# CrawlScript/tf_geometric

Measured on NVIDIA H100. Metric: edges/sec GCN+GAT fwd on 2.4M-node/123M-edge synthetic; %HBM roofline, higher is better.
Workload: dtype f32

## Files before the change

### include/tfgk.h

```cpp
#ifndef TFGK_H_
#define TFGK_H_

#include <stddef.h>
#include <stdint.h>

#ifdef __cplusplus
extern "C" {
#endif

#define TFGK_ABI_VERSION 7

enum tfgk_status {
    TFGK_OK = 0,
    TFGK_ERR_INVALID_ARGUMENT = 1,
    TFGK_ERR_CUDA = 2,
    TFGK_ERR_WORKSPACE = 3,
    TFGK_ERR_UNSUPPORTED = 4,
    TFGK_ERR_INDEX_OUT_OF_RANGE = 5
};

enum tfgk_reduce { TFGK_REDUCE_SUM = 0, TFGK_REDUCE_MEAN = 1, TFGK_REDUCE_MAX = 2 };
enum tfgk_act { TFGK_ACT_NONE = 0, TFGK_ACT_RELU = 1 };
enum tfgk_deg_power { TFGK_POW_INV_SQRT = 0, TFGK_POW_INV = 1 };
enum tfgk_heads_mode { TFGK_HEADS_SPLIT = 0, TFGK_HEADS_BROADCAST = 1, TFGK_HEADS_REDUCE = 2 };
// ... 57 lines not shown


int tfgk_spmm_f32(const int64_t *rowptr, const int32_t *col, const float *w,
                  const float *h, int64_t ldh, int32_t n_dst, int32_t D, int reduce,
                  float alpha, const float *addend, int64_t ld_addend, float beta,
                  const float *bias, int act,
                  float *out, int64_t ldo, const tfgk_plan *plan, void *stream);
int tfgk_spmm_bf16(const int64_t *rowptr, const int32_t *col, const float *w,
                   const uint16_t *h, int64_t ldh, int32_t n_dst, int32_t D, int reduce,
                   float alpha, const float *addend, int64_t ld_addend, float beta,
                   const float *bias, int act,
                   float *out, int64_t ldo, const tfgk_plan *plan, void *stream);
int tfgk_spmm_bf16_dual(const int64_t *rowptr, const int32_t *col, const float *w,
                        const uint16_t *h, int64_t ldh, int32_t n_dst, int32_t D, int reduce,
                        float alpha, const float *addend, int64_t ld_addend, float beta,
                        const float *bias, int act,
                        float *out, int64_t ldo, uint16_t *out_bf16, int64_t ldob,
                        const tfgk_plan *plan, void *stream);


int tfgk_segment_softmax_f32(const int64_t *rowptr, const float *score, int32_t n_seg, int32_t H,
                             float *out, void *stream);

int tfgk_gat_fused_f32(const int64_t *rowptr, const int32_t *col,
                       const float *Q, int64_t ldq, const float *K, int64_t ldk, const float *V, int64_t ldv,
                       int32_t N, int32_t H, int32_t dqk, int32_t dv, float scale, int split_value_heads,
                       const float *bias, int act, float *att, int write_att, float *out, int64_t ldo,
                       const tfgk_plan *plan, void *stream);
int tfgk_gat_fused_bf16(const int64_t *rowptr, const int32_t *col,
                        const float *Q, int64_t ldq, const uint16_t *K, int64_t ldk, const uint16_t *V, int64_t ldv,
                        int32_t N, int32_t H, int32_t dqk, int32_t dv, float scale, int split_value_heads,
                        const float *bias, int act, float *att, int write_att, float *out, int64_t ldo,
                        const tfgk_plan *plan, void *stream);


int tfgk_gemm_workspace_bytes(int32_t M, int32_t N, int32_t K, size_t *out_bytes);
int tfgk_gemm_f32(const float *A, int64_t lda, int transA, const float *B, int64_t ldb, int transB,
                  const float *bias, int act, float beta, int32_t M, int32_t N, int32_t K,
                  float *C, int64_t ldc, void *workspace, size_t workspace_bytes, void *stream);

typedef struct tfgk_proj_block {
    const float *B; int64_t ldb;
    int32_t ncols;
    int32_t transB;
    const float *bias;
    int act;
    float *C; int64_t ldc;
} tfgk_proj_block;
int tfgk_gemm_proj_f32(const float *const *A_parts, int32_t n_parts, int64_t part_rows, int64_t lda,
                       int32_t M, int32_t K, const tfgk_proj_block *blocks, int32_t n_blocks,
                       int32_t first_part, int32_t max_ctas, void *stream);
typedef struct tfgk_proj_block_out {
    const float *B; int64_t ldb;
    int32_t ncols;
    int32_t transB;
    const float *bias;
    int act;
    void *C; int64_t ldc;
    int32_t c_dtype;
} tfgk_proj_block_out;
int tfgk_gemm_proj_mixed(const float *const *A_parts, int32_t n_parts, int64_t part_rows, int64_t lda,
                         int32_t M, int32_t K, const tfgk_proj_block_out *blocks, int32_t n_blocks,
                         int32_t first_part, int32_t max_ctas, void *stream);
int tfgk_round_bf16(const float *src, int64_t lds, int32_t rows, int32_t cols, uint16_t *dst, int64_t ldd, void *stream);

#define TFGK_PEER_HANDLE_BYTES 64
// ... 125 lines not shown
```

### tf_geometric_b200/_ffi.py

```python
import ctypes
import os
import threading

_LIB_PATH = os.path.join(os.path.dirname(os.path.abspath(__file__)), "lib", "libtfgk.so")
_lock = threading.Lock()
_lib = None

ABI_VERSION = 7

OK = 0
ERR_INVALID_ARGUMENT, ERR_CUDA, ERR_WORKSPACE, ERR_UNSUPPORTED, ERR_INDEX_OUT_OF_RANGE = 1, 2, 3, 4, 5
REDUCE_SUM, REDUCE_MEAN, REDUCE_MAX = 0, 1, 2
ACT_NONE, ACT_RELU = 0, 1
POW_INV_SQRT, POW_INV = 0, 1
HEADS_SPLIT, HEADS_BROADCAST, HEADS_REDUCE = 0, 1, 2
FLAG_ALL, FLAG_UPPER, FLAG_MAPPED = 0, 1, 2
BERNOULLI_NONE, BERNOULLI_DROPOUT, BERNOULLI_KEEP = 0, 1, 2
SAMPLE_NO_PADDING, SAMPLE_PADDING, SAMPLE_HEAD = 0, 1, 2
NEG_UPPER, NEG_START = 0, 1
PAD_ROW_MAJOR, PAD_STEP_MAJOR = 0, 1
DTYPE_F32, DTYPE_BF16 = 0, 1

_i32, _i64, _f32, _int = ctypes.c_int32, ctypes.c_int64, ctypes.c_float, ctypes.c_int
_ptr, _size = ctypes.c_void_p, ctypes.c_size_t
# ... 1 lines not shown

SIGNATURES = {
    "tfgk_version": [],
    "tfgk_device_info": [ctypes.POINTER(_int)] * 3,
    "tfgk_self_loops_i32": [_ptr, _i64, _i32, _ptr, _ptr],
    "tfgk_self_loop_weights_f32": [_ptr, _i64, _i32, _f32, _ptr, _ptr],
    "tfgk_segment_count_i32": [_ptr, _i64, _i32, _ptr, _ptr],
    "tfgk_csr_workspace_bytes": [_i64, _i32, ctypes.POINTER(_size)],
    "tfgk_csr_build": [_ptr, _ptr, _i64, _i32, _i32, _ptr, _ptr, _ptr, _ptr, _size, _ptr],
    "tfgk_edge_unique_workspace_bytes": [_i64, _i32, ctypes.POINTER(_size)],
    "tfgk_edge_unique": [_ptr, _ptr, _i64, _i32, _ptr, _ptr, ctypes.POINTER(_i32), _ptr, _size, _ptr],
    "tfgk_directed_workspace_bytes": [_i64, ctypes.POINTER(_size)],
    "tfgk_directed_edges": [_ptr, _i64, _i64, _ptr, _i64, _ptr, ctypes.POINTER(_i32), _ptr, _size, _ptr],
    "tfgk_plan_capacity": [_i64, _i32, _i32, _i32, _i32, ctypes.POINTER(_i64), ctypes.POINTER(_i64)],
    "tfgk_plan_workspace_bytes": [_i32, ctypes.POINTER(_size)],
    "tfgk_plan_build": [_ptr, _i32, _i32, _i32, _i32, _ptr, _ptr, _ptr, _ptr, _ptr, _ptr, _ptr, _ptr, _i64, _i64,
                        ctypes.POINTER(_i32), _ptr, _size, _ptr],
    "tfgk_permute_f32": [_ptr, _ptr, _i64, _i32, _ptr, _ptr],
    "tfgk_unpermute_f32": [_ptr, _ptr, _i64, _i32, _ptr, _ptr],
    "tfgk_csr_rowsum_f32": [_ptr, _ptr, _i32, _ptr, _ptr],
    "tfgk_deg_inv_f32": [_ptr, _i32, _int, _ptr, _ptr],
    "tfgk_scale_edges_f32": [_ptr, _ptr, _ptr, _i64, _ptr, _ptr, _ptr, _ptr],
    "tfgk_spmm_f32": [_ptr, _ptr, _ptr, _ptr, _i64, _i32, _i32, _int, _f32, _ptr, _i64, _f32, _ptr, _int, _ptr, _i64,
                      _ptr, _ptr],
    "tfgk_spmm_bf16": [_ptr, _ptr, _ptr, _ptr, _i64, _i32, _i32, _int, _f32, _ptr, _i64, _f32, _ptr, _int, _ptr, _i64,
                       _ptr, _ptr],
    "tfgk_spmm_bf16_dual": [_ptr, _ptr, _ptr, _ptr, _i64, _i32, _i32, _int, _f32, _ptr, _i64, _f32, _ptr, _int, _ptr,
                            _i64, _ptr, _i64, _ptr, _ptr],
    "tfgk_segment_softmax_f32": [_ptr, _ptr, _i32, _i32, _ptr, _ptr],
    "tfgk_gat_fused_f32": [_ptr, _ptr, _ptr, _i64, _ptr, _i64, _ptr, _i64, _i32, _i32, _i32, _i32, _f32, _int, _ptr,
                           _int, _ptr, _int, _ptr, _i64, _ptr, _ptr],
    "tfgk_gat_fused_bf16": [_ptr, _ptr, _ptr, _i64, _ptr, _i64, _ptr, _i64, _i32, _i32, _i32, _i32, _f32, _int, _ptr,
                            _int, _ptr, _int, _ptr, _i64, _ptr, _ptr],
    "tfgk_gemm_workspace_bytes": [_i32, _i32, _i32, ctypes.POINTER(_size)],
    "tfgk_gemm_f32": [_ptr, _i64, _int, _ptr, _i64, _int, _ptr, _int, _f32, _i32, _i32, _i32, _ptr, _i64, _ptr, _size,
                      _ptr],
    "tfgk_gemm_proj_f32": [_ptr, _i32, _i64, _i64, _i32, _i32, _ptr, _i32, _i32, _i32, _ptr],
    "tfgk_gemm_proj_mixed": [_ptr, _i32, _i64, _i64, _i32, _i32, _ptr, _i32, _i32, _i32, _ptr],
    "tfgk_round_bf16": [_ptr, _i64, _i32, _i32, _ptr, _i64, _ptr],
    "tfgk_peer_alloc": [_size, ctypes.POINTER(_ptr)],
    "tfgk_peer_free": [_ptr],
    "tfgk_peer_export": [_ptr, _ptr],
    "tfgk_peer_open": [_ptr, ctypes.POINTER(_ptr)],
    "tfgk_peer_close": [_ptr],
    "tfgk_peer_barrier": [_ptr, _i32, _i32, _u32, _i32, _ptr],
    "tfgk_peer_pull": [_ptr, _ptr, _i64, _i32, _ptr],
    "tfgk_colsum_workspace_bytes": [_i64, _i32, ctypes.POINTER(_size)],
    "tfgk_colsum_f32": [_ptr, _i64, _i64, _i32, _ptr, _ptr, _size, _ptr],
    "tfgk_l2_normalize_f32": [_ptr, _i64, _i32, _i32, _ptr, _i64, _ptr],
    "tfgk_dropout_f32": [_ptr, _i64, _f32, _u64, _u32, _ptr, _ptr],
    "tfgk_spmm_heads_f32": [_ptr, _ptr, _ptr, _ptr, _ptr, _i64, _i32, _i32, _i32, _int, _f32, _u64, _u32, _f32, _ptr,
                            _int, _ptr, _i64, _ptr],
    "tfgk_gat_softmax_bwd_f32": [_ptr, _ptr, _ptr, _ptr, _i64, _ptr, _i64, _i32, _i32, _i32, _int, _f32, _u64, _u32,
                                 _ptr, _ptr],
    "tfgk_gat_fused_stats_f32": [_ptr, _ptr, _ptr, _i64, _ptr, _i64, _ptr, _i64, _i32, _i32, _i32, _i32, _f32, _ptr, _int,
                                 _ptr, _i64, _ptr, _ptr, _ptr],
    "tfgk_gat_bwd_prepare_f32": [_ptr, _i64, _ptr, _i64, _ptr, _int, _ptr, _i32, _i32, _i32, _ptr, _i64, _ptr],
    "tfgk_gat_bwd_dst_f32": [_ptr, _ptr, _ptr, _i64, _ptr, _i64, _ptr, _i64, _ptr, _i64, _i32, _i32, _i32, _f32, _ptr, _i64,
                             _ptr],
    "tfgk_gat_bwd_src_f32": [_ptr, _ptr, _ptr, _i64, _ptr, _i64, _ptr, _i64, _ptr, _i64, _i32, _i32, _i32, _f32, _ptr, _i64,
                             _ptr, _i64, _ptr],
    "tfgk_edge_flags_i32": [_ptr, _ptr, _i64, _int, _ptr, _ptr, _int, _f32, _u64, _u32, _ptr, _ptr],
    "tfgk_select_workspace_bytes": [_i64, ctypes.POINTER(_size)],
    "tfgk_select_flagged_i32": [_ptr, _i64, _ptr, ctypes.POINTER(_i64), _ptr, _size, _ptr],
    "tfgk_sort_keys_f32": [_ptr, _i64, _int, _ptr, _ptr],
    "tfgk_argsort_workspace_bytes": [_i64, ctypes.POINTER(_size)],
# ... 120 lines not shown
```

### tf_geometric_b200/csrc/gat.cu

```cuda
#include "common.cuh"
#include <stdlib.h>
#include <string.h>

namespace tfgk {

constexpr int kGatThreads = 256;
constexpr int kGatWarps = kGatThreads / 32;
constexpr int kMaxHeadsFast = 32;

__device__ __forceinline__ float4 ldg4(const float *p) { return __ldg(reinterpret_cast<const float4 *>(p)); }
__device__ __forceinline__ float4 ldg_row4(const float *p) { return ldg4(p); }
__device__ __forceinline__ float4 ldg_row4(const uint16_t *p) {
    const uint2 t = __ldg(reinterpret_cast<const uint2 *>(p));
    return make_float4(bf16_to_f32(t.x & 0xFFFFu), bf16_to_f32(t.x >> 16), bf16_to_f32(t.y & 0xFFFFu), bf16_to_f32(t.y >> 16));
}

struct GatParams {
    const int64_t *rowptr;
    const int32_t *col;
    const float *Q; int64_t ldq;
    const float *K; int64_t ldk;
    const float *V; int64_t ldv;
    const uint16_t *Kb, *Vb;
    int32_t N, H, dqk, dv;
    float scale;
    int split;
    const float *bias;
    int act;
    float *att;
    int write_att;
    float *out; int64_t ldo;
    int32_t n_tasks;
    const int32_t *task_row, *task_nrows;
    const int64_t *task_e0, *task_e1;
    const int32_t *task_slot;
    int32_t n_hubs;
    const int32_t *hub_row, *hub_slot0, *hub_nslots;
    float *scratch;
    float *stats;
};

template <int NCK, int NCV, int U>
__global__ void __launch_bounds__(kGatThreads) gat_fast_kernel(const GatParams p) {
    __shared__ float s_max[kGatWarps][kMaxHeadsFast];
    __shared__ float s_den[kGatWarps][kMaxHeadsFast];
    const int lane = threadIdx.x & 31, warp = threadIdx.x >> 5;
    const int64_t r = (int64_t)blockIdx.x * kGatWarps + warp;
    if (r >= p.N) return;
    const int H = p.H;
    const int A = H * p.dqk, VW = H * p.dv;
    const int lanes_per_head = p.dqk >> 2;
    const int64_t start = p.rowptr[r];
    const int deg = (int)(p.rowptr[r + 1] - start);
    float *att = p.att + start * H;

    int kcol[NCK];
    bool kok[NCK];
    float4 q[NCK];
    float mx[NCK];
#pragma unroll
    for (int k = 0; k < NCK; ++k) {
        kcol[k] = (lane + 32 * k) * 4;
        kok[k] = kcol[k] < A;
        q[k] = kok[k] ? ldg4(p.Q + r * p.ldq + kcol[k]) : make_float4(0.f, 0.f, 0.f, 0.f);
        mx[k] = -FLT_MAX;
    }
    for (int t = 0; t < deg; t += 32) {
        const int e = t + lane;
        const int my_c = e < deg ? ld_stream_i32(p.col + start + e) : 0;
        const int nb = min(32, deg - t);
        for (int j = 0; j < nb; j += U) {
            float4 kk[U][NCK];
// ... 595 lines not shown
        return TFGK_ERR_UNSUPPORTED;
    const size_t stage_pitch = ((size_t)4 * 2 * A * sizeof(T) + 127) & ~(size_t)127;
    const size_t smem = (size_t)kGatAsyncWarps * S * stage_pitch + (size_t)kGatAsyncWarps * S * 8;
    TFGK_CUDA(ensure_dynamic_smem(gat_tma4_kernel<S, T>, smem));
    const int64_t n_tasks = p.task_row ? p.n_tasks : ceil_div64(p.N, kGatAsyncRows);
    const unsigned blocks = (unsigned)ceil_div64(n_tasks, kGatAsyncWarps);
    gat_tma4_kernel<S, T><<<blocks, kGatAsyncWarps * 32, smem, st>>>(p);
    TFGK_LAUNCH_CHECK();
    if (p.task_row && p.n_hubs > 0) {
        gat_hub_fixup_kernel<<<(unsigned)ceil_div64(p.n_hubs, 8), 256, 0, st>>>(p);
        TFGK_LAUNCH_CHECK();
    }
    return TFGK_OK;
}

static int dispatch_gat_async(const GatParams &p, cudaStream_t st) {
    const char *g4 = getenv("TFGK_GAT_IMPL");
    if (!(g4 && g4[0] == 'a')) {
        const char *colon = g4 ? strchr(g4, ':') : nullptr;
        const int stages = colon ? atoi(colon + 1) : 2;
        const int rc = stages == 2 ? launch_gat_tma4<2>(p, st) : stages == 4 ? launch_gat_tma4<4>(p, st)
                                                                           : launch_gat_tma4<3>(p, st);
        if (rc != TFGK_ERR_UNSUPPORTED) return rc;
    }
    const char *cfg = getenv("TFGK_GAT_ASYNC_CFG");
    if (cfg && cfg[0] == '4' && cfg[2] == '2') return launch_gat_async<4, 2>(p, st);
    if (cfg && cfg[0] == '4' && cfg[2] == '3') return launch_gat_async<4, 3>(p, st);
    if (cfg && cfg[0] == '2' && cfg[2] == '4') return launch_gat_async<2, 4>(p, st);
    if (cfg && cfg[0] == '2' && cfg[2] == '2') return launch_gat_async<2, 2>(p, st);
    if (cfg && cfg[0] == '1' && cfg[2] == '4') return launch_gat_async<1, 4>(p, st);
    return launch_gat_async<2, 3>(p, st);
}

__device__ __forceinline__ float warp_sum(float v) {
#pragma unroll
    for (int off = 16; off > 0; off >>= 1) v += __shfl_xor_sync(0xffffffffu, v, off);
    return v;
}
__device__ __forceinline__ float warp_max(float v) {
#pragma unroll
    for (int off = 16; off > 0; off >>= 1) v = fmaxf(v, __shfl_xor_sync(0xffffffffu, v, off));
    return v;
}

__device__ __forceinline__ float ld_elem(const float *p) { return *p; }
__device__ __forceinline__ float ld_elem(const uint16_t *p) { return bf16_to_f32(*p); }

template <typename T>
__global__ void __launch_bounds__(kGatThreads) gat_generic_kernel(const GatParams p) {
    const T *Kt = sizeof(T) == 4 ? (const T *)p.K : (const T *)p.Kb;
    const T *Vt = sizeof(T) == 4 ? (const T *)p.V : (const T *)p.Vb;
    extern __shared__ float smem[];
    const int lane = threadIdx.x & 31, warp = threadIdx.x >> 5;
    const int64_t r = (int64_t)blockIdx.x * kGatWarps + warp;
    if (r >= p.N) return;
    const int H = p.H;
    float *s_max = smem + (size_t)warp * 2 * H;
    float *s_den = s_max + H;
    const int64_t start = p.rowptr[r];
    const int deg = (int)(p.rowptr[r + 1] - start);
    float *att = p.att + start * H;
    const int32_t *col = p.col + start;

    for (int h = lane; h < H; h += 32) s_max[h] = -FLT_MAX;
    __syncwarp();
    for (int e = 0; e < deg; ++e) {
// ... 240 lines not shown
    if (plan != nullptr && plan->n_tasks > 0) {
        if (plan->n_hubs > 0)
            TFGK_CHECK_ARG(plan->scratch != nullptr && plan->scratch_bytes >= (size_t)plan->n_slots * (VW + 64) * sizeof(float),
                           "gat: plan scratch too small (need %zu bytes)", (size_t)plan->n_slots * (VW + 64) * sizeof(float));
        p.n_tasks = plan->n_tasks; p.task_row = plan->task_row; p.task_nrows = plan->task_nrows;
        p.task_e0 = plan->task_e0; p.task_e1 = plan->task_e1; p.task_slot = plan->task_slot;
        p.n_hubs = plan->n_hubs; p.hub_row = plan->hub_row; p.hub_slot0 = plan->hub_slot0;
        p.hub_nslots = plan->hub_nslots; p.scratch = plan->scratch;
    }
    cudaStream_t st = as_stream(stream);
    const bool fast = split_value_heads && is_pow2(H) && H <= kMaxHeadsFast && dqk == dv && dqk % 4 == 0 &&
                      is_pow2(dqk / 4) && dqk <= 128 && A <= 512 && ldq % 4 == 0 && ldk % 4 == 0 && ldv % 4 == 0 &&
                      ldo % 4 == 0 && aligned16(Q) && aligned8(K) && aligned8(V) && aligned16(out) &&
                      (!bias || aligned16(bias));
    if (fast && A <= 128) {
        const int rc = launch_gat_tma4<3, uint16_t>(p, st);
        if (rc != TFGK_ERR_UNSUPPORTED) return rc;
    }
    if (fast) {
        switch ((A + 127) / 128) {
            case 1: return launch_gat_online<1, uint16_t>(p, st);
            case 2: return launch_gat_online<2, uint16_t>(p, st);
            case 3: return launch_gat_online<3, uint16_t>(p, st);
            default: return launch_gat_online<4, uint16_t>(p, st);
        }
    }
    if (att == nullptr) return set_error(TFGK_ERR_WORKSPACE, "gat: this shape needs the [E,H] attention scratch buffer");
    const size_t smem = (size_t)kGatWarps * 2 * H * sizeof(float);
    TFGK_CHECK_ARG(smem <= 48 * 1024, "gat: too many heads for the generic path (H=%d)", H);
    gat_generic_kernel<uint16_t><<<(unsigned)ceil_div64(N, kGatWarps), kGatThreads, smem, st>>>(p);
    TFGK_LAUNCH_CHECK();
    return TFGK_OK;
}
```

### tf_geometric_b200/nn/conv/gat.py

```python
import torch

from ... import ops, _structure, _rng, autograd
from ...sparse import as_sparse_features, project_features


def project(x, blocks):
    pieces = []
    for w, b, act, out in blocks:
        for c0 in range(0, w.shape[1], 128):
            c1 = min(c0 + 128, w.shape[1])
            pieces.append((w[:, c0:c1], None if b is None else b[c0:c1], act, out[:, c0:c1]))
    for i in range(0, len(pieces), 4):
        ops.gemm_proj(x, pieces[i:i + 4])


def gat(x, edge_index,
        query_kernel, query_bias, query_activation,
        key_kernel, key_bias, key_activation,
        kernel, bias=None, activation=None, num_heads=1,
        split_value_heads=True, edge_drop_rate=0.0, training=False, cache=None, return_attention=False, seed=None,
        message_dtype=None):
    bf16 = ops.message_dtype(message_dtype) is not None
    if bf16:
        if as_sparse_features(x) is not None:
            raise NotImplementedError("message_dtype=bfloat16 takes a dense x")
        if training and edge_drop_rate > 0.0:
            raise NotImplementedError("message_dtype=bfloat16 is for inference: attention dropout is not applied in bf16")
        if return_attention:
            raise NotImplementedError("message_dtype=bfloat16 does not return attention coefficients")
    edge_index = ops.as_device(edge_index, torch.int32)
    dev = edge_index.device
    x_sparse = as_sparse_features(x)
# ... 8 lines not shown
                raise NotImplementedError("return_attention is an inference-path extension")
            return _gat_training(x_sparse, csr, edge_index_used, query_kernel, query_bias, query_activation, key_kernel,
                                 key_bias, key_activation, kernel, bias, activation, num_heads, split_value_heads, drop_rate,
                                 _rng.resolve(seed) if drop_rate > 0.0 else 0)
        q_act, q_left = ops.activation_code(query_activation)
        k_act, k_left = ops.activation_code(key_activation)
        f32 = lambda t: None if t is None else ops.as_device(t, torch.float32, device=dev)
        Q = project_features(x_sparse, query_kernel, bias=f32(query_bias), act=q_act)
        K = project_features(x_sparse, key_kernel, bias=f32(key_bias), act=k_act)
        V = project_features(x_sparse, kernel)
        Q = q_left(Q) if q_left is not None else Q
        K = k_left(K) if k_left is not None else K
        act_code, leftover = ops.activation_code(activation)
        res = ops.gat_fused(csr, Q, K, V, num_heads, split_value_heads=split_value_heads, bias=f32(bias), act=act_code,
                            return_attention=return_attention)
        h, att = res if return_attention else (res, None)
        h = leftover(h) if leftover is not None else h
        return (h, ops.permute(att, csr.perm, inverse=True)) if return_attention else h
    if drop_rate > 0.0 or autograd.needs_grad(x, query_kernel, query_bias, key_kernel, key_bias, kernel, bias):
        if bf16:
            raise NotImplementedError("message_dtype=bfloat16 is for inference: no operand may require grad")
        if return_attention:
            raise NotImplementedError("return_attention is an inference-path extension")
        return _gat_training(x, csr, edge_index_used, query_kernel, query_bias, query_activation, key_kernel, key_bias,
                             key_activation, kernel, bias, activation, num_heads, split_value_heads, drop_rate,
                             _rng.resolve(seed) if drop_rate > 0.0 else 0)

    q_act, q_left = ops.activation_code(query_activation)
    k_act, k_left = ops.activation_code(key_activation)
    wq = ops.as_device(query_kernel, torch.float32, device=dev)
    wk = ops.as_device(key_kernel, torch.float32, device=dev)
    wv = ops.as_device(kernel, torch.float32, device=dev)
    a_units = wk.shape[1]
    Q = torch.empty((num_nodes, wq.shape[1]), dtype=torch.float32, device=dev)
    kv = torch.empty((num_nodes, a_units + wv.shape[1]), dtype=torch.bfloat16 if bf16 else torch.float32, device=dev)
    K, V = kv[:, :a_units], kv[:, a_units:]
    K_f32 = torch.empty((num_nodes, a_units), dtype=torch.float32, device=dev) if bf16 and k_left is not None else K
    project(x, [(wq, ops.as_device(query_bias, torch.float32, device=dev), q_act, Q),
                (wk, ops.as_device(key_bias, torch.float32, device=dev), k_act, K_f32),
                (wv, None, ops.ACT_NONE, V)])
    if q_left is not None:
        Q = q_left(Q)
    if k_left is not None:
        if K_f32 is K:
            K.copy_(k_left(K))
        else:
            ops.round_bf16(k_left(K_f32), out=K)

    act_code, leftover = ops.activation_code(activation)
    bias = None if bias is None else ops.as_device(bias, torch.float32, device=dev)
    res = ops.gat_fused(csr, Q, K, V, num_heads, split_value_heads=split_value_heads, bias=bias, act=act_code,
                        return_attention=return_attention)
    h, att = res if return_attention else (res, None)
    if leftover is not None:
        h = leftover(h)
    if return_attention:
        return h, ops.permute(att, csr.perm, inverse=True)
    return h


def _gat_training(x, csr, edge_index_used, query_kernel, query_bias, query_activation, key_kernel, key_bias,
                  key_activation, kernel, bias, activation, num_heads, split_value_heads, drop_rate, seed):
    sparse_x = as_sparse_features(x)
    dev = csr.col.device

    def dense(w, b, act):
        code, left = ops.activation_code(act)
        w = ops.as_device(w, torch.float32, device=dev)
        b = None if b is None else ops.as_device(b, torch.float32, device=dev)
        y = autograd.Dense.apply(x, w, b, code) if sparse_x is None else autograd.SparseMatmul.apply(w, b, sparse_x, code)
        return left(y) if left is not None else y

    Q = dense(query_kernel, query_bias, query_activation)
    K = dense(key_kernel, key_bias, key_activation)
    V = dense(kernel, None, None)
    act_code, leftover = ops.activation_code(activation)
    bias = None if bias is None else ops.as_device(bias, torch.float32, device=dev)
    h = autograd.GatAttention.apply(Q, K, V, bias, csr, edge_index_used, int(num_heads), bool(split_value_heads),
                                    act_code, drop_rate, seed)
    return leftover(h) if leftover is not None else h
```

### tf_geometric_b200/ops.py

```python
import ctypes

import numpy as np
import torch

from . import _ffi
from ._ffi import (REDUCE_SUM, REDUCE_MEAN, REDUCE_MAX, ACT_NONE, ACT_RELU, POW_INV_SQRT, POW_INV,
                   HEADS_SPLIT, HEADS_BROADCAST, HEADS_REDUCE, FLAG_ALL, FLAG_UPPER, FLAG_MAPPED,
                   BERNOULLI_NONE, BERNOULLI_DROPOUT, BERNOULLI_KEEP, SAMPLE_NO_PADDING, SAMPLE_PADDING, SAMPLE_HEAD,
                   NEG_UPPER, NEG_START, PAD_ROW_MAJOR, PAD_STEP_MAJOR)

_REDUCE_CODES = {"sum": REDUCE_SUM, "mean": REDUCE_MEAN, "max": REDUCE_MAX}


def _require_cuda():
    if not torch.cuda.is_available():
        raise RuntimeError("tf_geometric_b200 needs a CUDA device (H100 / sm_90a); there is no CPU fallback")


def default_device():
    _require_cuda()
    return torch.device("cuda", torch.cuda.current_device())


def as_device(x, dtype=None, device=None):
# ... 297 lines not shown
        raise ValueError("attention units ({}) and value units ({}) must be divisible by num_heads ({})".format(A, VW, H))
    dqk, dv = A // H, VW // H
    out_w = VW if split_value_heads else dv
    if out is None:
        out = torch.empty((N, out_w), dtype=torch.float32, device=Q.device)
    att = att_buffer
    if att is not None and att.numel() < csr.nnz * H:
        att = None
    if att is None and return_attention:
        att = torch.empty((csr.nnz, H), dtype=torch.float32, device=Q.device)
    if bias is not None:
        _check(bias, torch.float32, "bias")
    scale = float(np.sqrt(np.float32(dqk))) if scale is None else float(scale)

    plan = getattr(csr, "plan", None)
    plan_struct = plan.struct(VW + 64, Q.device) if plan is not None else None

    def launch(att_buf):
        _ffi.call("tfgk_gat_fused_bf16" if bf16 else "tfgk_gat_fused_f32", _p(csr.rowptr), _p(csr.col), _p(Q),
                  _row_major_2d(Q, "Q"), _p(K),
                  _row_major_2d(K, "K"), _p(V), _row_major_2d(V, "V"), N, H, dqk, dv, scale,
                  1 if split_value_heads else 0, _p(bias), act, _p(att_buf), 1 if return_attention else 0, _p(out),
                  _row_major_2d(out, "out"), ctypes.byref(plan_struct) if plan_struct is not None else None, _stream(Q))

    try:
        launch(att)
    except _ffi.TfgkError as err:
        if err.code != _ffi.ERR_WORKSPACE or att is not None:
            raise
        att = torch.empty((csr.nnz, H), dtype=torch.float32, device=Q.device)
        launch(att)
    if return_attention:
        return out, att[:csr.nnz]
    return out


def gat_fused_stats(csr, Q, K, V, num_heads, bias=None, act=ACT_NONE, scale=None):
    N, H = csr.n_rows, int(num_heads)
    A = Q.shape[1]
    if A % H or V.shape[1] != A or K.shape[1] != A:
        return None
    dqk = A // H
    scale = float(np.sqrt(np.float32(dqk))) if scale is None else float(scale)
    out = torch.empty((N, A), dtype=torch.float32, device=Q.device)
    stats = torch.empty((N, 2 * H), dtype=torch.float32, device=Q.device)
    plan = getattr(csr, "plan", None)
    plan_struct = plan.struct(A + 64, Q.device) if plan is not None else None
    try:
        _ffi.call("tfgk_gat_fused_stats_f32", _p(csr.rowptr), _p(csr.col), _p(Q), _row_major_2d(Q, "Q"), _p(K),
                  _row_major_2d(K, "K"), _p(V), _row_major_2d(V, "V"), N, H, dqk, dqk, scale, _p(bias), act, _p(out),
                  _row_major_2d(out, "out"), _p(stats), ctypes.byref(plan_struct) if plan_struct is not None else None, _stream(Q))
    except _ffi.TfgkError as err:
        if err.code != _ffi.ERR_UNSUPPORTED:
            raise
        return None
    return out, stats


def gat_backward_recompute(csr, csr_t, Q, K, V, G, Y, bias, act, stats, num_heads, scale):
    N, H = csr.n_rows, int(num_heads)
    A = Q.shape[1]
    dqk = A // H
    GS = torch.empty((N, A + 32), dtype=torch.float32, device=Q.device)
    dQ, dK, dV = torch.empty_like(Q), torch.empty_like(K), torch.empty_like(V)
    try:
        _ffi.call("tfgk_gat_bwd_prepare_f32", _p(G), _row_major_2d(G, "G"), _p(Y), _row_major_2d(Y, "Y"), _p(bias), act,
# ... 512 lines not shown
```

Measured before the change: 3.580 billion.

## Add sparsity-packed key table for GAT with ReLU keys to cut gather bytes

When keys pass through ReLU, a new pack kernel stores each node's V row followed by a nonzero bitmask and a compacted list of the nonzero K values, plus a per-node size byte. A new TMA-ring GAT kernel fetches only that variable-length slot per neighbor and rebuilds K from the mask with popcounts. The aim is to shrink the bytes gathered per edge, which dominate this bandwidth-bound kernel. It adds a pack pass, a per-edge size lookup, and decode work in the inner loop, and it only helps when ReLU leaves many keys at zero.

```diff
diff --git a/include/tfgk.h b/include/tfgk.h
--- a/include/tfgk.h
+++ b/include/tfgk.h
@@ -113,6 +113,12 @@
                         int32_t N, int32_t H, int32_t dqk, int32_t dv, float scale, int split_value_heads,
                         const float *bias, int act, float *att, int write_att, float *out, int64_t ldo,
                         const tfgk_plan *plan, void *stream);
+int tfgk_gat_pack_keys_f32(const float *K, int64_t ldk, int32_t N, int32_t A, float *table, int64_t ldt, uint8_t *ksize,
+                           void *stream);
+int tfgk_gat_fused_packed_f32(const int64_t *rowptr, const int32_t *col, const float *Q, int64_t ldq,
+                              const float *table, int64_t ldt, const uint8_t *ksize, int32_t N, int32_t H, int32_t dqk,
+                              float scale, const float *bias, int act, float *out, int64_t ldo,
+                              const tfgk_plan *plan, void *stream);
 
 
 int tfgk_gemm_workspace_bytes(int32_t M, int32_t N, int32_t K, size_t *out_bytes);
diff --git a/tf_geometric_b200/_ffi.py b/tf_geometric_b200/_ffi.py
--- a/tf_geometric_b200/_ffi.py
+++ b/tf_geometric_b200/_ffi.py
@@ -57,6 +57,9 @@
                            _int, _ptr, _int, _ptr, _i64, _ptr, _ptr],
     "tfgk_gat_fused_bf16": [_ptr, _ptr, _ptr, _i64, _ptr, _i64, _ptr, _i64, _i32, _i32, _i32, _i32, _f32, _int, _ptr,
                             _int, _ptr, _int, _ptr, _i64, _ptr, _ptr],
+    "tfgk_gat_pack_keys_f32": [_ptr, _i64, _i32, _i32, _ptr, _i64, _ptr, _ptr],
+    "tfgk_gat_fused_packed_f32": [_ptr, _ptr, _ptr, _i64, _ptr, _i64, _ptr, _i32, _i32, _i32, _f32, _ptr, _int, _ptr, _i64,
+                                  _ptr, _ptr],
     "tfgk_gemm_workspace_bytes": [_i32, _i32, _i32, ctypes.POINTER(_size)],
     "tfgk_gemm_f32": [_ptr, _i64, _int, _ptr, _i64, _int, _ptr, _int, _f32, _i32, _i32, _i32, _ptr, _i64, _ptr, _size,
                       _ptr],
diff --git a/tf_geometric_b200/csrc/gat.cu b/tf_geometric_b200/csrc/gat.cu
--- a/tf_geometric_b200/csrc/gat.cu
+++ b/tf_geometric_b200/csrc/gat.cu
@@ -38,6 +38,7 @@
     const int32_t *hub_row, *hub_slot0, *hub_nslots;
     float *scratch;
     float *stats;
+    const uint8_t *ksize = nullptr;
 };
 
 template <int NCK, int NCV, int U>
@@ -699,6 +700,234 @@
     return launch_gat_async<2, 3>(p, st);
 }
 
+constexpr int kPackWarps = 8;
+
+__global__ void __launch_bounds__(kPackWarps * 32) gat_pack_keys_kernel(const float *__restrict__ K, int64_t ldk, int32_t N,
+                                                                       int32_t A, float *__restrict__ table, int64_t ldt,
+                                                                       uint8_t *__restrict__ ksize) {
+    const int lane = threadIdx.x & 31;
+    const int64_t n = (int64_t)blockIdx.x * kPackWarps + (threadIdx.x >> 5);
+    if (n >= N) return;
+    const int ccol = lane * 4;
+    const float4 k = ccol < A ? __ldg(reinterpret_cast<const float4 *>(K + n * ldk + ccol)) : make_float4(0.f, 0.f, 0.f, 0.f);
+    const uint32_t nib = (__float_as_uint(k.x) != 0u ? 1u : 0u) | (__float_as_uint(k.y) != 0u ? 2u : 0u) |
+                         (__float_as_uint(k.z) != 0u ? 4u : 0u) | (__float_as_uint(k.w) != 0u ? 8u : 0u);
+    uint32_t word = nib << ((lane & 7) * 4);
+    word |= __shfl_xor_sync(0xffffffffu, word, 1);
+    word |= __shfl_xor_sync(0xffffffffu, word, 2);
+    word |= __shfl_xor_sync(0xffffffffu, word, 4);
+    const int cnt = __popc(nib);
+    int incl = cnt;
+#pragma unroll
+    for (int off = 1; off < 32; off <<= 1) {
+        const int t = __shfl_up_sync(0xffffffffu, incl, off);
+        if (lane >= off) incl += t;
+    }
+    const int total = __shfl_sync(0xffffffffu, incl, 31);
+    const uint32_t m0 = __shfl_sync(0xffffffffu, word, 0), m1 = __shfl_sync(0xffffffffu, word, 8);
+    const uint32_t m2 = __shfl_sync(0xffffffffu, word, 16), m3 = __shfl_sync(0xffffffffu, word, 24);
+    float *slot = table + n * ldt;
+    if (lane == 0) *reinterpret_cast<uint4 *>(slot + A) = make_uint4(m0, m1, m2, m3);
+    float *packed = slot + A + 4;
+    int o = incl - cnt;
+    if (nib & 1u) packed[o++] = k.x;
+    if (nib & 2u) packed[o++] = k.y;
+    if (nib & 4u) packed[o++] = k.z;
+    if (nib & 8u) packed[o] = k.w;
+    const int padded = (total + 3) & ~3;
+    if (lane < padded - total) packed[total + lane] = 0.0f;
+    if (lane == 0) ksize[n] = (uint8_t)((A + 4 + padded) / 4);
+}
+
+template <int S>
+__global__ void __launch_bounds__(kGatAsyncWarps * 32) gat_tma4_packed_kernel(const GatParams p) {
+    constexpr int U = 4, RPC = 32 / U;
+    static_assert(S - 1 <= RPC / 2, "the prologue must not reach the round that fetches chunk 1's copy sizes");
+    extern __shared__ __align__(128) uint8_t gat_pk_ring[];
+    const int lane = threadIdx.x & 31, warp = threadIdx.x >> 5;
+    const int A = p.H * p.dqk;
+    const uint32_t row_bytes = (uint32_t)A * 4u;
+    const uint32_t slot_bytes = (2u * row_bytes + 16u + 127u) & ~127u;
+    const uint32_t stage_bytes = (U * slot_bytes + 127u) & ~127u;
+    uint8_t *my_ring = gat_pk_ring + (size_t)warp * S * stage_bytes;
+    const uint32_t ring_addr = (uint32_t)__cvta_generic_to_shared(my_ring);
+    uint64_t *bars = reinterpret_cast<uint64_t *>(gat_pk_ring + (size_t)kGatAsyncWarps * S * stage_bytes) + warp * S;
+    const uint32_t bar0 = (uint32_t)__cvta_generic_to_shared(bars);
+    if (lane == 0) {
+#pragma unroll
+        for (int i = 0; i < S; ++i) asm volatile("mbarrier.init.shared::cta.b64 [%0], 1;" ::"r"(bar0 + 8 * i));
+        asm volatile("fence.mbarrier_init.release.cluster;" ::: "memory");
+    }
+    __syncwarp();
+    const int64_t task = (int64_t)blockIdx.x * kGatAsyncWarps + warp;
+    int64_t r0, r1, e_begin, e_stop;
+    int slot = -1;
+    if (p.task_row != nullptr) {
+        if (task >= p.n_tasks) return;
+        r0 = p.task_row[task];
+        r1 = r0 + p.task_nrows[task];
+        e_begin = p.task_e0[task];
+        e_stop = p.task_e1[task];
+        slot = p.task_slot[task];
+    } else {
+        r0 = task * kGatAsyncRows;
+        if (r0 >= p.N) return;
+        r1 = min((int64_t)p.N, r0 + kGatAsyncRows);
+        e_begin = p.rowptr[r0];
+        e_stop = p.rowptr[r1];
+    }
+    const int64_t rp_hi = p.rowptr[min(r0 + lane + 1, r1)];
+    const int n_edges = (int)(e_stop - e_begin);
+    const int n_rounds = (n_edges + U - 1) / U;
+    const int lanes_per_head = p.dqk >> 2;
+    const int ccol = lane * 4;
+    const bool cok = ccol < A;
+    const int sh = (lane & 7) * 4, wsel = lane >> 3;
+    const uint32_t below_lo = (1u << sh) - 1u;
+    const uint32_t bm0 = wsel > 0 ? ~0u : wsel == 0 ? below_lo : 0u, bm1 = wsel > 1 ? ~0u : wsel == 1 ? below_lo : 0u;
+    const uint32_t bm2 = wsel > 2 ? ~0u : wsel == 2 ? below_lo : 0u, bm3 = wsel == 3 ? below_lo : 0u;
+
+    int64_t r = r0;
+    int row_end = slot >= 0 ? 0x7fffffff : (int)(__shfl_sync(0xffffffffu, rp_hi, 0) - e_begin);
+    float4 q = cok ? ldg4(p.Q + r * p.ldq + ccol) : make_float4(0.f, 0.f, 0.f, 0.f);
+    float4 q_next = (cok && r + 1 < r1) ? ldg4(p.Q + (r + 1) * p.ldq + ccol) : make_float4(0.f, 0.f, 0.f, 0.f);
+    float mx = -FLT_MAX, den = 0.0f, a0 = 0.f, a1 = 0.f, a2 = 0.f, a3 = 0.f;
+    float4 bias = make_float4(0.f, 0.f, 0.f, 0.f);
+    if (p.bias && cok) bias = ldg4(p.bias + ccol);
+
+    auto finalize_row = [&]() {
+        if (cok) {
+            const float inv = 1.0f / (den + 1e-8f);
+            float4 o;
+            o.x = apply_act(a0 * inv + bias.x, p.act);
+            o.y = apply_act(a1 * inv + bias.y, p.act);
+            o.z = apply_act(a2 * inv + bias.z, p.act);
+            o.w = apply_act(a3 * inv + bias.w, p.act);
+            *reinterpret_cast<float4 *>(p.out + r * p.ldo + ccol) = o;
+        }
+        mx = -FLT_MAX; den = 0.0f; a0 = a1 = a2 = a3 = 0.0f;
+        ++r;
+        q = q_next;
+        if (r < r1) {
+            row_end = (int)(__shfl_sync(0xffffffffu, rp_hi, (int)(r - r0)) - e_begin);
+            if (cok && r + 1 < r1) q_next = ldg4(p.Q + (r + 1) * p.ldq + ccol);
+        }
+    };
+    auto load_chunk = [&](int c) {
+        const int e = c * 32 + lane;
+        return e < n_edges ? ld_stream_i32(p.col + e_begin + e) : 0;
+    };
+    auto load_sizes = [&](int ci) { return (int)__ldg(p.ksize + ci); };
+    auto issue = [&](int g, int ci, int si) {
+        if (g < n_rounds) {
+            const int base = (g % RPC) * U;
+            const int valid = min(U, n_edges - g * U);
+            const int src = base + (lane < U ? lane : 0);
+            const int c = __shfl_sync(0xffffffffu, ci, src);
+            const uint32_t bytes = 16u * (uint32_t)__shfl_sync(0xffffffffu, si, src);
+            uint32_t tx = lane < valid ? bytes : 0u;
+            tx += __shfl_xor_sync(0xffffffffu, tx, 1);
+            tx += __shfl_xor_sync(0xffffffffu, tx, 2);
+            const uint32_t bar = bar0 + 8 * (uint32_t)(g % S);
+            if (lane == 0)
+                asm volatile("mbarrier.arrive.expect_tx.shared::cta.b64 _, [%0], %1;" ::"r"(bar), "r"(tx) : "memory");
+            if (lane < valid)
+                asm volatile("cp.async.bulk.shared::cluster.global.mbarrier::complete_tx::bytes [%0], [%1], %2, [%3];"
+                             ::"r"(ring_addr + (uint32_t)(g % S) * stage_bytes + (uint32_t)lane * slot_bytes),
+                             "l"(p.K + (int64_t)c * p.ldk), "r"(bytes), "r"(bar) : "memory");
+        }
+    };
+
+    int ca = load_chunk(0), cb = load_chunk(1);
+    int sa = load_sizes(ca), sb = 0;
+#pragma unroll
+    for (int g = 0; g < S - 1; ++g) issue(g, ca, sa);
+
+    for (int g = 0; g < n_rounds; ++g) {
+        __syncwarp();
+        {
+            const int gn = g + S - 1;
+            const int k = gn / RPC;
+            if (gn % RPC == RPC / 2) {
+                if (k & 1) sa = load_sizes(ca); else sb = load_sizes(cb);
+            }
+            issue(gn, (k & 1) ? cb : ca, (k & 1) ? sb : sa);
+        }
+        gat_mbar_wait(bar0 + 8 * (uint32_t)(g % S), (uint32_t)(g / S) & 1u);
+        const uint8_t *sbuf = my_ring + (size_t)(g % S) * stage_bytes;
+        float4 kr[U];
+#pragma unroll
+        for (int u = 0; u < U; ++u) {
+            kr[u] = make_float4(0.f, 0.f, 0.f, 0.f);
+            if (g * U + u < n_edges && cok) {
+                const uint8_t *sl = sbuf + (size_t)u * slot_bytes + row_bytes;
+                const uint4 m = *reinterpret_cast<const uint4 *>(sl);
+                const uint32_t bits = *reinterpret_cast<const uint32_t *>(sl + 4 * wsel) >> sh;
+                int o = __popc(m.x & bm0) + __popc(m.y & bm1) + __popc(m.z & bm2) + __popc(m.w & bm3);
+                const float *pk = reinterpret_cast<const float *>(sl + 16);
+                if (bits & 1u) kr[u].x = pk[o++];
+                if (bits & 2u) kr[u].y = pk[o++];
+                if (bits & 4u) kr[u].z = pk[o++];
+                if (bits & 8u) kr[u].w = pk[o];
+            }
+        }
+#pragma unroll
+        for (int u = 0; u < U; ++u) {
+            const int e = g * U + u;
+            if (e < n_edges) {
+                while (e == row_end) finalize_row();
+                const float4 kk = kr[u];
+                float4 vv = make_float4(0.f, 0.f, 0.f, 0.f);
+                if (cok) vv = *reinterpret_cast<const float4 *>(sbuf + (size_t)u * slot_bytes + ccol * 4);
+                float d = __fmul_rn(q.x, kk.x);
+                d = fmaf(q.y, kk.y, d);
+                d = fmaf(q.z, kk.z, d);
+                d = fmaf(q.w, kk.w, d);
+                for (int off = 1; off < lanes_per_head; off <<= 1) d += __shfl_xor_sync(0xffffffffu, d, off);
+                const float s = __fdiv_rn(d, p.scale);
+                const bool up = s > mx;
+                const float t = expf(up ? mx - s : s - mx);
+                const float corr = up ? t : 1.0f, pe = up ? 1.0f : t;
+                mx = up ? s : mx;
+                den = fmaf(den, corr, pe);
+                a0 = fmaf(a0, corr, pe * vv.x);
+                a1 = fmaf(a1, corr, pe * vv.y);
+                a2 = fmaf(a2, corr, pe * vv.z);
+                a3 = fmaf(a3, corr, pe * vv.w);
+            }
+        }
+        if ((g + S) % RPC == 0) {
+            const int dead = (g + S) / RPC - 1;
+            if (dead & 1) cb = load_chunk(dead + 2); else ca = load_chunk(dead + 2);
+        }
+    }
+    if (slot >= 0) {
+        float *dst = p.scratch + (int64_t)slot * (A + 64);
+        if (cok) *reinterpret_cast<float4 *>(dst + ccol) = make_float4(a0, a1, a2, a3);
+        dst[A + lane] = mx;
+        dst[A + 32 + lane] = den;
+        return;
+    }
+    while (r < r1) finalize_row();
+}
+
+template <int S>
+static int launch_gat_packed(const GatParams &p, cudaStream_t st) {
+    const size_t slot_bytes = ((size_t)8 * p.H * p.dqk + 16 + 127) & ~(size_t)127;
+    const size_t stage_pitch = (4 * slot_bytes + 127) & ~(size_t)127;
+    const size_t smem = (size_t)kGatAsyncWarps * S * stage_pitch + (size_t)kGatAsyncWarps * S * 8;
+    TFGK_CUDA(ensure_dynamic_smem(gat_tma4_packed_kernel<S>, smem));
+    const int64_t n_tasks = p.task_row ? p.n_tasks : ceil_div64(p.N, kGatAsyncRows);
+    const unsigned blocks = (unsigned)ceil_div64(n_tasks, kGatAsyncWarps);
+    gat_tma4_packed_kernel<S><<<blocks, kGatAsyncWarps * 32, smem, st>>>(p);
+    TFGK_LAUNCH_CHECK();
+    if (p.task_row && p.n_hubs > 0) {
+        gat_hub_fixup_kernel<<<(unsigned)ceil_div64(p.n_hubs, 8), 256, 0, st>>>(p);
+        TFGK_LAUNCH_CHECK();
+    }
+    return TFGK_OK;
+}
+
 __device__ __forceinline__ float warp_sum(float v) {
 #pragma unroll
     for (int off = 16; off > 0; off >>= 1) v += __shfl_xor_sync(0xffffffffu, v, off);
@@ -1005,3 +1234,59 @@
     TFGK_LAUNCH_CHECK();
     return TFGK_OK;
 }
+
+extern "C" int tfgk_gat_pack_keys_f32(const float *K, int64_t ldk, int32_t N, int32_t A, float *table, int64_t ldt,
+                                      uint8_t *ksize, void *stream) {
+    TFGK_CHECK_ARG(N >= 0 && A >= 4 && A <= 128 && A % 4 == 0, "gat_pack_keys: bad size (N=%d A=%d; A must be 4..128, a multiple of 4)",
+                   N, A);
+    TFGK_CHECK_ARG(ldk >= A && ldk % 4 == 0 && ldt >= 2 * A + 4 && ldt % 16 == 0,
+                   "gat_pack_keys: leading dimensions (ldk=%lld, ldt=%lld; ldt a multiple of 16, at least 2A + 4)",
+                   (long long)ldk, (long long)ldt);
+    if (N == 0) return TFGK_OK;
+    TFGK_CHECK_ARG(K && table && ksize, "gat_pack_keys: null pointer");
+    TFGK_CHECK_ARG(aligned16(K) && aligned16(table), "gat_pack_keys: K and table must be 16-byte aligned");
+    gat_pack_keys_kernel<<<(unsigned)ceil_div64(N, kPackWarps), kPackWarps * 32, 0, as_stream(stream)>>>(K, ldk, N, A, table,
+                                                                                                         ldt, ksize);
+    TFGK_LAUNCH_CHECK();
+    return TFGK_OK;
+}
+
+extern "C" int tfgk_gat_fused_packed_f32(const int64_t *rowptr, const int32_t *col, const float *Q, int64_t ldq,
+                                         const float *table, int64_t ldt, const uint8_t *ksize, int32_t N, int32_t H,
+                                         int32_t dqk, float scale, const float *bias, int act, float *out, int64_t ldo,
+                                         const tfgk_plan *plan, void *stream) {
+    TFGK_CHECK_ARG(N >= 0 && H >= 1 && dqk >= 1, "gat_packed: bad size (N=%d H=%d dqk=%d)", N, H, dqk);
+    TFGK_CHECK_ARG(act == TFGK_ACT_NONE || act == TFGK_ACT_RELU, "gat_packed: unknown activation %d", act);
+    TFGK_CHECK_ARG(scale > 0.0f, "gat_packed: scale must be positive");
+    const int A = H * dqk;
+    if (!(is_pow2(H) && H <= kMaxHeadsFast && dqk % 4 == 0 && is_pow2(dqk / 4) && A <= 128))
+        return set_error(TFGK_ERR_UNSUPPORTED, "gat_packed: H must be a power of two <= 32, dqk / 4 a power of two, H * dqk <= 128");
+    TFGK_CHECK_ARG(ldq >= A && ldo >= A && ldt >= 2 * A + 4, "gat_packed: leading dimension too small");
+    if (N == 0) return TFGK_OK;
+    TFGK_CHECK_ARG(rowptr && col && Q && table && ksize && out, "gat_packed: null pointer");
+    if (ldq % 4 || ldo % 4 || ldt % 16 || !aligned16(Q) || !aligned16(out) || !aligned16(table) || (bias && !aligned16(bias)))
+        return set_error(TFGK_ERR_UNSUPPORTED, "gat_packed: Q, out, bias and table need 16-byte aligned rows, slots of a multiple of 64 bytes");
+
+    GatParams p;
+    p.rowptr = rowptr; p.col = col;
+    p.Q = Q; p.ldq = ldq; p.K = table; p.ldk = ldt; p.V = table; p.ldv = ldt; p.Kb = nullptr; p.Vb = nullptr;
+    p.N = N; p.H = H; p.dqk = dqk; p.dv = dqk; p.scale = scale; p.split = 1;
+    p.bias = bias; p.act = act; p.att = nullptr; p.write_att = 0; p.out = out; p.ldo = ldo;
+    p.n_tasks = 0; p.task_row = nullptr; p.task_nrows = nullptr; p.task_e0 = nullptr; p.task_e1 = nullptr;
+    p.task_slot = nullptr; p.n_hubs = 0; p.hub_row = nullptr; p.hub_slot0 = nullptr; p.hub_nslots = nullptr; p.scratch = nullptr;
+    p.stats = nullptr;
+    p.ksize = ksize;
+    if (plan != nullptr && plan->n_tasks > 0) {
+        if (plan->n_hubs > 0)
+            TFGK_CHECK_ARG(plan->scratch != nullptr && plan->scratch_bytes >= (size_t)plan->n_slots * (A + 64) * sizeof(float),
+                           "gat_packed: plan scratch too small (need %zu bytes)", (size_t)plan->n_slots * (A + 64) * sizeof(float));
+        p.n_tasks = plan->n_tasks; p.task_row = plan->task_row; p.task_nrows = plan->task_nrows;
+        p.task_e0 = plan->task_e0; p.task_e1 = plan->task_e1; p.task_slot = plan->task_slot;
+        p.n_hubs = plan->n_hubs; p.hub_row = plan->hub_row; p.hub_slot0 = plan->hub_slot0;
+        p.hub_nslots = plan->hub_nslots; p.scratch = plan->scratch;
+    }
+    cudaStream_t st = as_stream(stream);
+    const char *env = getenv("TFGK_GAT_PACKED_STAGES");
+    const int stages = env ? atoi(env) : 2;
+    return stages == 3 ? launch_gat_packed<3>(p, st) : stages == 4 ? launch_gat_packed<4>(p, st) : launch_gat_packed<2>(p, st);
+}
diff --git a/tf_geometric_b200/nn/conv/gat.py b/tf_geometric_b200/nn/conv/gat.py
--- a/tf_geometric_b200/nn/conv/gat.py
+++ b/tf_geometric_b200/nn/conv/gat.py
@@ -1,3 +1,5 @@
+import os
+
 import torch
 
 from ... import ops, _structure, _rng, autograd
@@ -72,6 +74,24 @@
     wk = ops.as_device(key_kernel, torch.float32, device=dev)
     wv = ops.as_device(kernel, torch.float32, device=dev)
     a_units = wk.shape[1]
+    act_code, leftover = ops.activation_code(activation)
+    bias = None if bias is None else ops.as_device(bias, torch.float32, device=dev)
+    if not bf16 and not return_attention and k_act == ops.ACT_RELU and k_left is None and x.is_cuda and \
+            _packed_keys_shape(wq, wk, wv, bias, num_heads, split_value_heads) and \
+            os.environ.get("TFGK_GAT_KEYS", "packed") != "dense":
+        Q = torch.empty((num_nodes, a_units), dtype=torch.float32, device=dev)
+        K = torch.empty((num_nodes, a_units), dtype=torch.float32, device=dev)
+        table, sizes = ops.packed_key_table(num_nodes, a_units, dev)
+        project(x, [(wq, ops.as_device(query_bias, torch.float32, device=dev), q_act, Q),
+                    (wk, ops.as_device(key_bias, torch.float32, device=dev), k_act, K),
+                    (wv, None, ops.ACT_NONE, table[:, :a_units])])
+        if q_left is not None:
+            Q = q_left(Q)
+        ops.gat_pack_keys(K, table, sizes)
+        del K
+        h = ops.gat_fused_packed(csr, Q, table, sizes, num_heads, bias=bias, act=act_code)
+        return leftover(h) if leftover is not None else h
+
     Q = torch.empty((num_nodes, wq.shape[1]), dtype=torch.float32, device=dev)
     kv = torch.empty((num_nodes, a_units + wv.shape[1]), dtype=torch.bfloat16 if bf16 else torch.float32, device=dev)
     K, V = kv[:, :a_units], kv[:, a_units:]
@@ -87,8 +107,6 @@
         else:
             ops.round_bf16(k_left(K_f32), out=K)
 
-    act_code, leftover = ops.activation_code(activation)
-    bias = None if bias is None else ops.as_device(bias, torch.float32, device=dev)
     res = ops.gat_fused(csr, Q, K, V, num_heads, split_value_heads=split_value_heads, bias=bias, act=act_code,
                         return_attention=return_attention)
     h, att = res if return_attention else (res, None)
@@ -97,6 +115,14 @@
     if return_attention:
         return h, ops.permute(att, csr.perm, inverse=True)
     return h
+
+
+def _packed_keys_shape(wq, wk, wv, bias, num_heads, split_value_heads):
+    H, A = int(num_heads), wk.shape[1]
+    if not split_value_heads or wq.shape[1] != A or wv.shape[1] != A or A > 128 or H < 1 or H > 32 or H & (H - 1) or A % H:
+        return False
+    d4 = (A // H) // 4
+    return (A // H) % 4 == 0 and d4 >= 1 and d4 & (d4 - 1) == 0 and (bias is None or bias.data_ptr() % 16 == 0)
 
 
 def _gat_training(x, csr, edge_index_used, query_kernel, query_bias, query_activation, key_kernel, key_bias,
diff --git a/tf_geometric_b200/ops.py b/tf_geometric_b200/ops.py
--- a/tf_geometric_b200/ops.py
+++ b/tf_geometric_b200/ops.py
@@ -353,6 +353,48 @@
         launch(att)
     if return_attention:
         return out, att[:csr.nnz]
+    return out
+
+
+def gat_packed_width(units):
+    return -(-(2 * int(units) + 4) // 32) * 32
+
+
+def packed_key_table(num_nodes, units, device):
+    table = torch.empty((int(num_nodes), gat_packed_width(units)), dtype=torch.float32, device=device)
+    sizes = torch.empty((int(num_nodes),), dtype=torch.uint8, device=device)
+    return table, sizes
+
+
+def gat_pack_keys(K, table, sizes):
+    if not (K.is_cuda and K.dtype == torch.float32 and K.dim() == 2):
+        raise TypeError("gat_pack_keys: K must be a 2-D float32 CUDA tensor")
+    _check(sizes, torch.uint8, "sizes")
+    N, A = K.shape
+    if table.dtype != torch.float32 or table.shape[0] != N or sizes.shape[0] != N:
+        raise ValueError("gat_pack_keys: table and sizes must have {} rows".format(N))
+    _ffi.call("tfgk_gat_pack_keys_f32", _p(K), _row_major_2d(K, "K"), N, A, _p(table), _row_major_2d(table, "table"),
+              _p(sizes), _stream(K))
+    return table, sizes
+
+
+def gat_fused_packed(csr, Q, table, sizes, num_heads, bias=None, act=ACT_NONE, out=None, scale=None):
+    _check(sizes, torch.uint8, "sizes")
+    if not (Q.is_cuda and Q.dtype == torch.float32 and table.is_cuda and table.dtype == torch.float32):
+        raise TypeError("gat_fused_packed: Q and table must be float32 CUDA tensors")
+    N, H, A = csr.n_rows, int(num_heads), Q.shape[1]
+    if A % H:
+        raise ValueError("attention units ({}) must be divisible by num_heads ({})".format(A, H))
+    if out is None:
+        out = torch.empty((N, A), dtype=torch.float32, device=Q.device)
+    if bias is not None:
+        _check(bias, torch.float32, "bias")
+    scale = float(np.sqrt(np.float32(A // H))) if scale is None else float(scale)
+    plan = getattr(csr, "plan", None)
+    plan_struct = plan.struct(A + 64, Q.device) if plan is not None else None
+    _ffi.call("tfgk_gat_fused_packed_f32", _p(csr.rowptr), _p(csr.col), _p(Q), _row_major_2d(Q, "Q"), _p(table),
+              _row_major_2d(table, "table"), _p(sizes), N, H, A // H, scale, _p(bias), act, _p(out), _row_major_2d(out, "out"),
+              ctypes.byref(plan_struct) if plan_struct is not None else None, _stream(Q))
     return out
 
 
```

After: 3.902 billion, median of 6. +9.0%, better.
